# td-kwj-zp2023/webgpu-msm-bls12-377

Hardware: AMD Instinct MI355X
Metric: ms per 2^20 BLS12-377 G1 MSM (lower is better)
Workload: dtype u32 (29-bit limbs, 64-bit accumulate)

## Files before the change

webgpu-msm-bls12-377_amd/csrc/common.hpp:

```cpp
#pragma once
#include <stdint.h>

#include "../../include/msm377.h"

#ifndef MSM_HD
#if defined(__HIPCC__)
#include <hip/hip_runtime.h>
#define MSM_HD __host__ __device__ __forceinline__
#else
#define MSM_HD inline __attribute__((always_inline))
#endif
#endif

namespace msm377 {

constexpr uint32_t NB = 32768;
constexpr uint32_t NBIN = NB + 1;
constexpr uint32_t RP = NBIN + 1;
constexpr uint32_t PT_WORDS = 52;
constexpr uint32_t BKT_WORDS = 64;
constexpr uint32_t MAX_SORT_BLOCKS = 256;
constexpr uint32_t TREE_LEVELS = 15;
constexpr uint32_t SEG_MIN = 16;
constexpr uint32_t SEG_MAX = 128;
// ... 12 lines not shown
static_assert(short_windows(253, 15) == MSM377_NUM_WINDOWS && short_windows(253, NARROW_LOG) == NARROW_EVEN_WINDOWS, "at full width: the window counts of the main and the narrow path");

constexpr uint32_t NRANGE = 256;
constexpr uint32_t KRANGE = NB / NRANGE;
constexpr uint32_t KEY_TRACKED = 0x80000000u;
constexpr uint32_t KEY_UNSIGNED = 0x40000000u;
constexpr uint32_t SMALL_SORT_MAX = 1u << 16;
constexpr uint32_t SMALL_BINS_MAX = (1u << 12) + 1;
struct SortElem {
  uint32_t idx_sign;
  uint32_t key;
};
struct SortElem4 {
  uint32_t v;
};
constexpr uint32_t SORT_IDX_BITS = 23, SORT_SUB_BITS = 8;
constexpr uint64_t SORT_PACKED_MAX_COLUMNS = 1ull << SORT_IDX_BITS;
static_assert(SORT_IDX_BITS + SORT_SUB_BITS + 1 == 32, "index, sub and sign fill the 32-bit element");
static_assert(KRANGE < (1u << SORT_SUB_BITS), "sub = 0..KRANGE fits its field");
MSM_HD SortElem4 sort_pack(uint32_t idx, uint32_t sign, uint32_t sub) { return SortElem4{(sign << 31) | (sub << SORT_IDX_BITS) | idx}; }
MSM_HD uint32_t sort_sub(SortElem4 e) { return (e.v >> SORT_IDX_BITS) & ((1u << SORT_SUB_BITS) - 1u); }
MSM_HD uint32_t sort_idx_sign(SortElem4 e) { return e.v & ~(((1u << SORT_SUB_BITS) - 1u) << SORT_IDX_BITS); }
MSM_HD uint32_t range_first_key(uint32_t rg, uint32_t shift) { return rg * (KRANGE >> shift); }
inline uint32_t sort_elem_bytes(uint64_t columns, bool wide) { return (!wide && columns <= SORT_PACKED_MAX_COLUMNS) ? 4u : 8u; }

struct WorkItem {
  uint32_t row;
  uint32_t seg;
};
constexpr uint32_t META_BLOCK_WORDS = 2 * SEG_BINS + 4 + MSM377_NUM_WINDOWS;
constexpr size_t SLOT_WORDS = (size_t)MAX_WINDOW_SLOTS * MSM377_G1_PARTIAL_POINTS * MSM377_G1_POINT_WORDS;

constexpr uint32_t AFF_THREADS = 256, AFF_K = 8, AFF_BLOCK_POINTS = AFF_THREADS * AFF_K;
constexpr uint32_t AFF_STASH_WORDS = 52;
inline uint32_t affine_blocks(uint64_t n) { return (uint32_t)((n + AFF_BLOCK_POINTS - 1) / AFF_BLOCK_POINTS); }

constexpr uint32_t ACC_FLAG_WORD = 4;
constexpr uint32_t EVEN_FROM = 13;
constexpr uint32_t even_offset(uint32_t w) { return 16 * w - (w > EVEN_FROM ? w - EVEN_FROM : 0u); }
static_assert(even_offset(13) == 208 && even_offset(14) == 223 && even_offset(15) == 238 && even_offset(16) == 253, "13 x 16 + 3 x 15 = 253 bits");
constexpr uint32_t WIDE_BITS = MSM377_WIDE_WINDOW_BITS;
constexpr uint32_t WIDE_LOG = 19;
constexpr uint32_t WIDE_WINDOWS = 13;
constexpr uint32_t WIDE_FULL = 6;
constexpr uint32_t wide_width(uint32_t w) { return w < WIDE_FULL ? WIDE_BITS : WIDE_BITS - 1; }
constexpr uint32_t wide_offset(uint32_t w) { return w <= WIDE_FULL ? WIDE_BITS * w : WIDE_BITS * WIDE_FULL + (WIDE_BITS - 1) * (w - WIDE_FULL); }
static_assert(wide_offset(WIDE_WINDOWS - 1) == 234 && wide_offset(WIDE_WINDOWS - 1) + wide_width(WIDE_WINDOWS - 1) == 253, "the windows cover a 253-bit scalar");
constexpr uint32_t WIDE_NRANGE = 4096;
constexpr uint32_t WIDE_POINTS = WIDE_LOG + 1;
static_assert((1u << WIDE_LOG) == WIDE_NRANGE * KRANGE, "ranges of KRANGE keys cover the wide bucket set");
static_assert((1u << WIDE_LOG) <= MSM377_NUM_WINDOWS * NB, "the wide bucket set fits the main path's bucket, row and work-list buffers");
static_assert(WIDE_POINTS * 1 <= MAX_WINDOW_SLOTS * MSM377_G1_PARTIAL_POINTS, "the wide window record fits a partial-record slot");

constexpr uint32_t G1_REC_WORDS = 32;
constexpr uint32_t GLV_WINDOWS = MSM377_GLV_WINDOWS;

}
```

webgpu-msm-bls12-377_amd/csrc/consts_gen.hpp:

```cpp
#pragma once
#include <stdint.h>

namespace msm377 {

struct G1Consts {
static constexpr int NL = 13;
static constexpr int RS = 14;
static constexpr uint32_t KP2[13] = {0x20000002u, 0x308bffffu, 0x20000041u, 0x2d7510bfu, 0x290002e0u, 0x222fba08u, 0x3c78f79au, 0x3cc03d43u, 0x363445b2u, 0x26ca1492u, 0x231d82dfu, 0x3f1443aau, 0x35c748c1u};
static constexpr uint32_t KP6[13] = {0x20000006u, 0x31a3ffffu, 0x200000c6u, 0x285f323fu, 0x3b0008a3u, 0x268f2e1au, 0x356ae6d0u, 0x3640b7cdu, 0x229cd11au, 0x345e3dbau, 0x2958889fu, 0x3d3ccb00u, 0xa155da47u};
static constexpr uint32_t KP4W3[13] = {0x60000004u, 0x6117fffdu, 0x60000082u, 0x7aea217du, 0x720005bfu, 0x645f740fu, 0x78f1ef33u, 0x79807a86u, 0x6c688b64u, 0x6d942924u, 0x663b05bdu, 0x7e288753u, 0x6b8e9182u};
static constexpr uint32_t MOD2[13] = {0x00000002u, 0x108c0000u, 0x00000042u, 0x0d7510c0u, 0x090002e1u, 0x022fba09u, 0x1c78f79bu, 0x1cc03d44u, 0x163445b3u, 0x06ca1493u, 0x031d82e0u, 0x1f1443abu, 0x35c748c2u};
static constexpr uint32_t MOD4[13] = {0x00000004u, 0x01180000u, 0x00000085u, 0x1aea2180u, 0x120005c2u, 0x045f7412u, 0x18f1ef36u, 0x19807a89u, 0x0c688b67u, 0x0d942927u, 0x063b05c0u, 0x1e288756u, 0x6b8e9185u};
static constexpr uint32_t MOD[13] = {0x00000001u, 0x08460000u, 0x00000021u, 0x16ba8860u, 0x14800170u, 0x1117dd04u, 0x0e3c7bcdu, 0x1e601ea2u, 0x1b1a22d9u, 0x03650a49u, 0x118ec170u, 0x0f8a21d5u, 0x1ae3a461u};
static constexpr uint32_t ONE[13] = {0x19eaf730u, 0x171ffffeu, 0x0d714cf8u, 0x044e31d8u, 0x1eb6e262u, 0x0bfad163u, 0x00d46e9cu, 0x10b6ddbfu, 0x13b9cbddu, 0x075782afu, 0x03bd1d8au, 0x1557cab6u, 0x15742a14u};
static constexpr uint32_t R2[13] = {0x1c14cc5cu, 0x07b8df46u, 0x04c74875u, 0x0d6832fau, 0x05f4afc1u, 0x11ea1ee5u, 0x09265a5fu, 0x09fa84f9u, 0x12f6f558u, 0x18644b2bu, 0x1caa9452u, 0x011db07du, 0x0ef492d1u};
static constexpr uint32_t GEN_X[13] = {0x1ce797d8u, 0x17fe48a3u, 0x1f3536a5u, 0x0dc25c2bu, 0x1e104e6bu, 0x1eae505du, 0x0e4e1ad8u, 0x06034dddu, 0x1a0c4bbau, 0x1a00fcf3u, 0x0d60a010u, 0x0f8b893du, 0x0350969fu};
static constexpr uint32_t GEN_Y[13] = {0x1cad4e90u, 0x1ad19703u, 0x05ab84b1u, 0x0efc4cdcu, 0x0ea1dd3du, 0x16ca39d3u, 0x1a70f7f0u, 0x07c10e01u, 0x119daf26u, 0x1ea6b705u, 0x1f2b10a9u, 0x09c00e16u, 0x157eb1a4u};
static constexpr uint32_t B3[13] = {0x0dc0e58eu, 0x14d3fffcu, 0x0853e6a7u, 0x1f7584c9u, 0x1324a444u, 0x01c0ba22u, 0x0604543au, 0x15645bf8u, 0x04f91de4u, 0x0f3c737bu, 0x0819d5beu, 0x00f31c77u, 0x0a95357bu};
static constexpr uint32_t BETA[13] = {0x1c8a7893u, 0x0b7d08f2u, 0x06b88506u, 0x162aa2edu, 0x1c5fdf80u, 0x11b95a22u, 0x03b86dd7u, 0x1191f770u, 0x10701220u, 0x1501c11fu, 0x1cee88bbu, 0x118d05ecu, 0x06f2fa26u};
static constexpr uint32_t TE_S[13] = {0x08449ac2u, 0x16bc6341u, 0x1f27346eu, 0x003fa706u, 0x16341794u, 0x0e03035eu, 0x1f0a2ed9u, 0x0c4c0908u, 0x1a0645ffu, 0x0dd41749u, 0x078fb647u, 0x1b5db1c4u, 0x1660c39du};
static constexpr uint32_t TE_CS[13] = {0x0c11be99u, 0x0aedb353u, 0x14c24473u, 0x198caca0u, 0x1709c799u, 0x1d5780a3u, 0x0f7d035fu, 0x121a0ad5u, 0x0cb37c72u, 0x1eef061fu, 0x0da87607u, 0x1503504au, 0x001d4357u};
static constexpr uint32_t TE_2D[13] = {0x114806b1u, 0x04ef4e0du, 0x07df1bf4u, 0x01a7deddu, 0x07626a98u, 0x061c00c8u, 0x1b3f730cu, 0x037d439du, 0x1c957daau, 0x096f1594u, 0x098747aeu, 0x19dba77fu, 0x03dbbc1fu};
static constexpr uint32_t TE_INV_D[13] = {0x1235813du, 0x1a6958e8u, 0x0842a642u, 0x0ccc3277u, 0x130f1cf2u, 0x012ee262u, 0x18833f19u, 0x19503cf9u, 0x194bf957u, 0x1e6caec8u, 0x17390a9eu, 0x1ab4def3u, 0x10163111u};
static constexpr uint32_t TE_SR[13] = {0x15c55a01u, 0x1bcf91e7u, 0x09410bb6u, 0x1b458877u, 0x1f3e06b9u, 0x1b799510u, 0x13b0477au, 0x166cebb0u, 0x16d99580u, 0x1e1e3f33u, 0x141fe804u, 0x0e8bd79bu, 0x07643ddau};
static constexpr uint32_t TE_CSR[13] = {0x0e6d2f3fu, 0x083d0045u, 0x1a1e3b24u, 0x1500eeabu, 0x0b424b4au, 0x0f2708c5u, 0x13fa6b3eu, 0x0e79a13bu, 0x1bd40692u, 0x15a4c276u, 0x029c52e0u, 0x17b697c3u, 0x042252f1u};
static constexpr uint32_t TE_SBR[13] = {0x17d64e6fu, 0x0c701d9au, 0x1096c343u, 0x0f28269au, 0x1dd6a07bu, 0x0d2d995au, 0x0b7abebcu, 0x01039476u, 0x0754bb75u, 0x17ed77a6u, 0x10ad99d1u, 0x0295f06bu, 0x0eee0d30u};
static constexpr uint32_t TE_CSBR[13] = {0x101ae105u, 0x14e123bau, 0x0c011795u, 0x1e120f1bu, 0x013e4a5du, 0x00f36391u, 0x05460450u, 0x1213a321u, 0x02049adcu, 0x1e46b54eu, 0x03ec2c28u, 0x0719faedu, 0x04062136u};
static constexpr uint32_t CHK_RHS_RAW[13] = {0x1b151a26u, 0x1887416bu, 0x12ef1461u, 0x11a8bb6fu, 0x1402fb5bu, 0x08e38166u, 0x0355b0e6u, 0x1233c29au, 0x08a7a722u, 0x009a7635u, 0x1e0bf740u, 0x0c427686u, 0x0fde33f9u};
static constexpr uint32_t IMPORT_MONT384[13] = {0x00400000u, 0x00000000u, 0x00000000u, 0x00000000u, 0x00000000u, 0x00000000u, 0x00000000u, 0x00000000u, 0x00000000u, 0x00000000u, 0x00000000u, 0x00000000u, 0x00000000u};
static constexpr uint32_t TO64[13] = {0x1fffff68u, 0x166fffffu, 0x1fffec40u, 0x013f06ffu, 0x13ff2514u, 0x19d4c53eu, 0x0c167df6u, 0x16edcf8cu, 0x087b4e97u, 0x1c01e427u, 0x133d256fu, 0x05fbe934u, 0x08d6661eu};
static constexpr int PM2_NW = 12;
static constexpr uint32_t PM2_W[12] = {0xffffffffu, 0x8508bfffu, 0x30000000u, 0x170b5d44u, 0xba094800u, 0x1ef3622fu, 0x00f5138fu, 0x1a22d9f3u, 0x6ca1493bu, 0xc63b05c0u, 0x17c510eau, 0x01ae3a46u};
static constexpr uint32_t GEN_WIRE[24] = {0xb21be9efu, 0xeab9b16eu, 0xffcd394eu, 0xd5481512u, 0xbd37cb5cu, 0x188282c8u, 0xaa9d41bbu, 0x85951e2cu, 0xbf87ff54u, 0xc8fc6225u, 0xfe740a67u, 0x008848deu, 0x559c8ea6u, 0xfd82de55u, 0x34a9591au, 0xc2fe3d36u, 0x4fb82305u, 0x6d182ad4u, 0xca3e52d9u, 0xbd7fb348u, 0x30afeec4u, 0x1f674f5du, 0xc5102effu, 0x01914a69u};
};

struct GlvConsts {
static constexpr uint32_t LAMBDA[4] = {0x00000000u, 0x0a118000u, 0x90000001u, 0x452217ccu};
static constexpr uint32_t MU[9] = {0x7b820d29u, 0x5cc5a03bu, 0x6f25c6b5u, 0x3366fc87u, 0xaf90182cu, 0x7f72ed32u, 0x9fd37160u, 0xb3f7aa96u, 0x00000003u};
};

struct EdConsts {
static constexpr int NL = 9;
static constexpr int RS = 9;
static constexpr uint32_t KP2[9] = {0x20000002u, 0x2117ffffu, 0x20000084u, 0x29dbfb3fu, 0x36002b34u, 0x2d1e5c36u, 0x2ab305a1u, 0x37a68b28u, 0x002556c9u};
static constexpr uint32_t KP6[9] = {0x20000006u, 0x2347ffffu, 0x2000018eu, 0x3d93f1bfu, 0x2200819eu, 0x275b14a6u, 0x201910e6u, 0x26f3a17bu, 0x0070045fu};
static constexpr uint32_t KP4W3[9] = {0x60000004u, 0x622ffffdu, 0x60000107u, 0x73b7f67du, 0x6c005667u, 0x7a3cb86cu, 0x75660b41u, 0x6f4d164fu, 0x004aad92u};
static constexpr uint32_t MOD2[9] = {0x00000002u, 0x01180000u, 0x00000085u, 0x09dbfb40u, 0x16002b35u, 0x0d1e5c37u, 0x0ab305a2u, 0x17a68b29u, 0x002556cau};
static constexpr uint32_t MOD4[9] = {0x00000004u, 0x02300000u, 0x0000010au, 0x13b7f680u, 0x0c00566au, 0x1a3cb86fu, 0x15660b44u, 0x0f4d1652u, 0x004aad95u};
static constexpr uint32_t MOD[9] = {0x00000001u, 0x108c0000u, 0x00000042u, 0x14edfda0u, 0x1b00159au, 0x068f2e1bu, 0x155982d1u, 0x0bd34594u, 0x0012ab65u};
static constexpr uint32_t ONE[9] = {0x1ffffe4au, 0x1077ffffu, 0x1fff8e31u, 0x10d0103fu, 0x0ddb0965u, 0x07071c5cu, 0x18da2e10u, 0x0486f3a3u, 0x000ec090u};
static constexpr uint32_t R2[9] = {0x0615ebc3u, 0x1d9b570cu, 0x191f15fbu, 0x00f6d3e2u, 0x15ede530u, 0x0fadbc68u, 0x0428942fu, 0x06a15030u, 0x000c9478u};
static constexpr uint32_t ED_D[9] = {0x1febc5efu, 0x0eb3ffffu, 0x1abe9217u, 0x003be85fu, 0x0004720du, 0x05dec129u, 0x1512d0bbu, 0x09975a7cu, 0x000242cau};
static constexpr uint32_t ED_2D[9] = {0x1fd78bdeu, 0x1d67ffffu, 0x157d242eu, 0x0077d0bfu, 0x0008e41au, 0x0bbd8252u, 0x0a25a176u, 0x132eb4f9u, 0x00048594u};
static constexpr uint32_t GEN_X[9] = {0x0cca7270u, 0x0e8466dcu, 0x18ea02c5u, 0x0a3e1cacu, 0x0d288491u, 0x08fdc59du, 0x02b87f4fu, 0x00370735u, 0x0002b438u};
static constexpr uint32_t GEN_Y[9] = {0x19e7fa03u, 0x1cbf8d15u, 0x147cb8ddu, 0x0759f755u, 0x096d8529u, 0x0350b3f2u, 0x14b6ec89u, 0x0691eb12u, 0x000577c8u};
static constexpr uint32_t TE_2D[9] = {0x1fd78bdeu, 0x1d67ffffu, 0x157d242eu, 0x0077d0bfu, 0x0008e41au, 0x0bbd8252u, 0x0a25a176u, 0x132eb4f9u, 0x00048594u};
static constexpr uint32_t IMPORT_MONT256[9] = {0x00000020u, 0x00000000u, 0x00000000u, 0x00000000u, 0x00000000u, 0x00000000u, 0x00000000u, 0x00000000u, 0x00000000u};
static constexpr uint32_t TO64[9] = {0x1ffffff3u, 0x08e3ffffu, 0x1ffffc9fu, 0x0fea1edfu, 0x00fee725u, 0x0abaa896u, 0x0a745b60u, 0x06457773u, 0x000d4bdau};
static constexpr int PM2_NW = 8;
static constexpr uint32_t PM2_W[8] = {0xffffffffu, 0x0a117fffu, 0xd0000001u, 0x59aa76feu, 0x5c37b001u, 0x60b44d1eu, 0x9a2ca556u, 0x12ab655eu};
// ... 41 lines not shown
```

webgpu-msm-bls12-377_amd/csrc/context.hip:

```cpp
#include "context.hpp"

#include <string.h>

#include <algorithm>
#include <new>

#include "sequencer.hpp"

using namespace msm377;

hipError_t Resources::alloc(void** p, size_t bytes) {
  const hipError_t rc = hipMalloc(p, bytes);
  if (rc == hipSuccess) device.push_back(*p);
  else *p = nullptr;
  return rc;
}
hipError_t Resources::alloc_pinned(void** p, size_t bytes, unsigned flags) {
  const hipError_t rc = hipHostMalloc(p, bytes, flags);
  if (rc == hipSuccess) pinned.push_back(*p);
  else *p = nullptr;
  return rc;
}
hipError_t Resources::event(hipEvent_t* e, unsigned flags) {
  const hipError_t rc = hipEventCreateWithFlags(e, flags);
// ... 54 lines not shown
  ctx->tail_pool.wait_limit_ns = (int64_t)knobs.tail_wait_ms * 1000000ll;
  ctx->tail_pool.numa_local = knobs.tail_numa;
  Resources& own = ctx->own;
  const uint64_t cap = max_points;
  int prio_least = 0, prio_greatest = 0;
  bool ok = hipSetDevice(device) == hipSuccess;
  if (ok && hipDeviceGetStreamPriorityRange(&prio_least, &prio_greatest) != hipSuccess) prio_least = prio_greatest = 0;
  ok = ok && own.stream(&ctx->stream, &prio_greatest) == hipSuccess && own.stream(&ctx->stream2, &prio_least) == hipSuccess &&
       own.event(&ctx->bases_ready, hipEventDisableTiming) == hipSuccess;
  auto dalloc = [&](void** p, size_t bytes) { ok = ok && own.alloc(p, bytes) == hipSuccess; };
  if (!borrows_bases) dalloc((void**)&ctx->d_raw_points, cap * 96);
  dalloc((void**)&ctx->d_raw_scalars, cap * 32);
  if (!borrows_bases) dalloc((void**)&ctx->d_bases, 2 * cap * G1_REC_WORDS * 4);
  const uint64_t wcap = std::max<uint64_t>((uint64_t)MSM377_NUM_WINDOWS * cap, (uint64_t)NARROW_EVEN_WINDOWS * std::min<uint64_t>(cap, SMALL_SORT_MAX));
  dalloc((void**)&ctx->d_digits, wcap * 2);
  dalloc((void**)&ctx->d_range_counts, (size_t)NRANGE * MAX_SORT_BLOCKS * 4);
  dalloc((void**)&ctx->d_region_base, (size_t)MSM377_NUM_WINDOWS * (NRANGE + 1) * 4);
  dalloc((void**)&ctx->d_sort_temp, cap * MSM377_NUM_WINDOWS * sizeof(SortElem));
  dalloc((void**)&ctx->d_row_ptr, (size_t)MSM377_NUM_WINDOWS * RP * 4);
  dalloc((void**)&ctx->d_val_idx, wcap * 4);
  dalloc((void**)&ctx->d_buckets, (size_t)MSM377_NUM_WINDOWS * BKT_WORDS * NB * 4);
  dalloc((void**)&ctx->d_partials, (size_t)2 * SLOT_WORDS * 4);
  const uint64_t extra_items = std::max<uint64_t>((uint64_t)MSM377_NUM_WINDOWS * cap / SEG_MIN, (uint64_t)NARROW_EVEN_WINDOWS * std::min<uint64_t>(cap, SMALL_SORT_MAX) / NARROW_SEG) + 2;
  dalloc((void**)&ctx->d_work, ((size_t)MSM377_NUM_WINDOWS * NB + extra_items) * sizeof(WorkItem));
  dalloc((void**)&ctx->d_work_meta, (size_t)META_BLOCK_WORDS * 4);
  dalloc((void**)&ctx->d_row_ovf_base, (size_t)MSM377_NUM_WINDOWS * NB * 4);
  dalloc((void**)&ctx->d_split_rows, (size_t)MSM377_NUM_WINDOWS * NB * 4);
  dalloc((void**)&ctx->d_ovf, (size_t)extra_items * BKT_WORDS * 4);
  AffineConvert& aff = ctx->aff;
  ZeroCopyOut& zc = ctx->zc;
  const size_t aff_blocks = (size_t)affine_blocks(cap) + 1;
  dalloc((void**)&aff.d_count, 64);
  ok = ok && hipMemset(aff.d_count, 0, 64) == hipSuccess;
  dalloc((void**)&aff.d_stash, (size_t)affine_blocks(cap) * AFF_BLOCK_POINTS * AFF_STASH_WORDS * 4);
  dalloc((void**)&aff.d_trees, aff_blocks * 2 * AFF_THREADS * 13 * 4);
  const unsigned host_flags = hipHostMallocMapped | hipHostMallocCoherent;
  ok = ok && own.alloc_pinned((void**)&aff.h_prod, aff_blocks * 48, host_flags) == hipSuccess &&
       own.alloc_pinned((void**)&aff.h_inv, aff_blocks * 48, host_flags) == hipSuccess &&
       own.alloc_pinned((void**)&aff.h_flag, 64, host_flags) == hipSuccess &&
       hipHostGetDevicePointer((void**)&aff.dm_prod, aff.h_prod, 0) == hipSuccess &&
       hipHostGetDevicePointer((void**)&aff.dm_inv, aff.h_inv, 0) == hipSuccess &&
       hipHostGetDevicePointer((void**)&aff.dm_flag, aff.h_flag, 0) == hipSuccess &&
       own.event(&aff.up_done, hipEventDisableTiming) == hipSuccess;
  if (ok) aff.scratch.resize(aff_blocks);
  dalloc((void**)&ctx->d_err, 4 * sizeof(int));
  ok = ok && own.alloc_pinned((void**)&ctx->h_partials, (size_t)2 * SLOT_WORDS * 4, host_flags) == hipSuccess &&
       hipHostGetDevicePointer((void**)&zc.dm_partials, ctx->h_partials, 0) == hipSuccess &&
       own.alloc_pinned((void**)&zc.h_flag, 64, host_flags) == hipSuccess &&
       hipHostGetDevicePointer((void**)&zc.dm_flag, zc.h_flag, 0) == hipSuccess;
  if (ok) memset(zc.h_flag, 0, 64);
  dalloc((void**)&zc.d_count, 64);
  ok = ok && hipMemset(zc.d_count, 0, 64) == hipSuccess;
  ok = ok && own.alloc_pinned((void**)&ctx->h_err, 2 * sizeof(int)) == hipSuccess;
  for (int k = 0; ok && k < 2; k++) ok = ok && own.event(&ctx->done_ev[k], hipEventDisableTiming) == hipSuccess;
  for (int s = 0; ok && s < MSM377_NUM_STAGES; s++)
    for (int k = 0; k < 2; k++) ok = ok && own.event(&ctx->ev[s][k]) == hipSuccess;
  if (!ok) {
    ctx_destroy(ctx);
    return MSM377_ENOMEM;
  }
  *out = ctx;
  return MSM377_OK;
}

void ctx_destroy(msm377_ctx* ctx) {
  if (!ctx) return;
  ctx->tail_pool.shutdown();
// ... 66 lines not shown
```

webgpu-msm-bls12-377_amd/csrc/context.hpp:

```cpp
#pragma once
#include <hip/hip_runtime.h>

#include <functional>
#include <string>
#include <vector>

#include "common.hpp"
#include "fp64_host.hpp"
#include "knobs.hpp"
#include "tail_pool.hpp"

using msm377::SortElem;
using msm377::WorkItem;
using msm377::TailPool;
using msm377::Fp64;
using msm377::MAX_WINDOW_SLOTS;
using msm377::NARROW_SEG;
using msm377::Knobs;

struct Resources {
  std::vector<void*> device, pinned;
  std::vector<hipEvent_t> events;
  std::vector<hipStream_t> streams;
  hipError_t alloc(void** p, size_t bytes);
// ... 58 lines not shown
  uint32_t k = 0;
  int width = 0;
  uint32_t* tables = nullptr;
  bool valid() const { return k != 0; }
};

struct WideBuffers {
  uint32_t* digits = nullptr;
  SortElem* temp = nullptr;
  uint32_t* counts = nullptr;
  uint64_t cap = 0;
  bool ensure(Resources& own, uint64_t n, size_t counts_words);
  void release(Resources& own);
};

struct StageLayout {
  bool valid = false;
  msm377_stage_info info = {};
  const void* d_digits = nullptr;
  const uint32_t* d_key_max = nullptr;
  uint32_t coord_words = 16, limbs = 13;
};

struct BasesLayout {
  bool valid = false;
  msm377_bases_info info = {};
  const uint32_t* d_records = nullptr;
  const uint32_t* d_flagged = nullptr;
};


struct AffineConvert {
  uint32_t* d_stash = nullptr;
  uint32_t* d_trees = nullptr;
  uint32_t* h_prod = nullptr;
  uint32_t* h_inv = nullptr;
  uint32_t* h_flag = nullptr;
  uint32_t *dm_prod = nullptr, *dm_inv = nullptr, *dm_flag = nullptr;
  uint32_t* d_count = nullptr;
  hipEvent_t up_done = nullptr;
  std::vector<Fp64::El> scratch;
};

struct ZeroCopyOut {
  bool active = false;
  uint32_t out_seq = 0;
  uint32_t acc_seq = 0;
  uint32_t* h_flag = nullptr;
  uint32_t* dm_flag = nullptr;
  uint32_t* dm_partials = nullptr;
  uint32_t* d_count = nullptr;
};

struct NativeImport {
  uint64_t cap = 0;
  uint8_t* d_native = nullptr;
  uint32_t* d_inf_mask = nullptr;
  hipEvent_t import_done = nullptr;
  size_t mask_words() const { return (size_t)(((cap + 31) / 32 + 3) & ~3ull); }
  size_t points_bytes() const { return ((size_t)cap * 104 + 15) & ~(size_t)15; }
  uint8_t* native_points() const { return d_native; }
  uint8_t* native_scalars() const { return d_native + points_bytes(); }
};

struct HostStaging {
  uint8_t* h_stage = nullptr;
// ... 87 lines not shown
```

webgpu-msm-bls12-377_amd/csrc/kernels/convert.hpp:

```cpp
#pragma once
#include "../curves.hpp"

namespace msm377 {
namespace {


__global__ void __launch_bounds__(256) k_clear_words(uint32_t* __restrict__ a, uint32_t na, uint32_t* __restrict__ b, uint32_t nb) {
  for (uint32_t i = threadIdx.x; i < na; i += 256) a[i] = 0;
  for (uint32_t i = threadIdx.x; i < nb; i += 256) b[i] = 0;
}

template <class CV>
__global__ void __launch_bounds__(256) k_convert_bases(const uint32_t* __restrict__ raw, uint32_t* __restrict__ bases, uint64_t n, int* __restrict__ err) {
  uint64_t i = (uint64_t)blockIdx.x * 256 + threadIdx.x;
  if (i >= n) return;
  uint32_t w[CV::RAW_WORDS];
  load_words16(raw + i * CV::RAW_WORDS, w, CV::RAW_WORDS / 4);
  uint32_t o[CV::REC_WORDS];
  if (CV::convert(w, o)) atomicOr(err, ERR_TE_CONVERT);
  uint4* dst = reinterpret_cast<uint4*>(bases + i * CV::REC_WORDS);
#pragma unroll
  for (int k = 0; k < (int)CV::REC_WORDS / 4; k++) dst[k] = make_uint4(o[4 * k], o[4 * k + 1], o[4 * k + 2], o[4 * k + 3]);
}

// ... 12 lines not shown
  const uint32_t* raw;
  __device__ __forceinline__ bool load(uint64_t i, Fp::El& n1, Fp::El& n2, Fp::El& z) const {
    using K = G1Consts;
    uint32_t w[24];
    load_words16(raw + i * 24, w, 6);
    const Fp::El xr = Fp::from_words<12>(w), yr = Fp::from_words<12>(w + 12);
    const Fp::El u = Fp::add_lz(Fp::mul_lz(xr, Fp::from_const(K::TE_SR)), Fp::from_const(K::TE_S));
    const Fp::El v = Fp::mul_lz(yr, Fp::from_const(K::TE_SR));
    const Fp::El cu = Fp::csub(Fp::norm(Fp::add_lz(Fp::mul_lz(xr, Fp::from_const(K::TE_CSR)), Fp::from_const(K::TE_CS))), K::MOD);
    const Fp::El up = Fp::add_lz(u, Fp::one());
    z = Fp::mul_lz(up, v);
    n1 = Fp::mul_lz(up, cu);
    n2 = Fp::norm(Fp::add_kp_sub_sub2(z, K::KP4W3, Fp::zero(), v));
    return Te377::is_zero_mod_p(z);
  }
};
struct AffDoublingSource {
  const uint32_t* prev;
  uint32_t bits;
  __device__ __forceinline__ bool load(uint64_t i, Fp::El& n1, Fp::El& n2, Fp::El& z) const {
    Te377::Ext p = Te377::from_base_affine(TeAffBase::load_base(prev, (uint32_t)i), false);
    bool bad = false;
#pragma unroll 1
    for (uint32_t k = 0; k < bits; k++) {
      p = Te377::add(p, p);
      bad |= Te377::is_bad(p);
    }
    n1 = Fp::canon(p.x);
    n2 = Fp::canon(p.y);
    z = Fp::canon(p.z);
    return bad;
  }
};
template <class SRC>
__global__ void __launch_bounds__(AFF_THREADS, 4) k_affine_up(SRC src, uint64_t n, uint32_t* __restrict__ stash,
                                                              uint32_t* __restrict__ trees, uint32_t* __restrict__ block_prod, uint32_t* __restrict__ host_flag, uint32_t* __restrict__ dev_count,
                                                              int* __restrict__ err, uint32_t prio) {
  if (prio) __builtin_amdgcn_s_setprio(3);
  using K = G1Consts;
  __shared__ uint32_t tree[2 * AFF_THREADS][13];
  const uint32_t tid = threadIdx.x, blk = blockIdx.x;
  const uint64_t base = (uint64_t)blk * AFF_BLOCK_POINTS + tid;
  bool bad = false;
  Fp::El c = Fp::one();
#pragma unroll 1
  for (uint32_t j = 0; j < AFF_K; j++) {
    const uint64_t i = base + (uint64_t)j * AFF_THREADS;
    if (i >= n) break;
    Fp::El n1, n2, z;
    if (src.load(i, n1, n2, z)) {
      bad = true;
      z = Fp::one();
    }
    uint32_t o[AFF_STASH_WORDS];
    put13(o, n1);
    put13(o + 13, n2);
    put13(o + 26, z);
    put13(o + 39, c);
    uint4* dst = reinterpret_cast<uint4*>(stash) + ((size_t)blk * AFF_K + j) * (AFF_STASH_WORDS / 4) * AFF_THREADS + tid;
#pragma unroll
    for (int k = 0; k < (int)AFF_STASH_WORDS / 4; k++) dst[(size_t)k * AFF_THREADS] = make_uint4(o[4 * k], o[4 * k + 1], o[4 * k + 2], o[4 * k + 3]);
    c = Fp::mul_lz(c, z);
  }
  if (bad) atomicOr(err, ERR_TE_CONVERT);
  put13(tree[AFF_THREADS + tid], c);
  for (uint32_t size = AFF_THREADS / 2; size >= 1; size >>= 1) {
    __syncthreads();
    if (tid < size) put13(tree[size + tid], Fp::mul_lz(get13(tree[2 * (size + tid)]), get13(tree[2 * (size + tid) + 1])));
  }
  __syncthreads();
  uint32_t* out = trees + (size_t)blk * (2 * AFF_THREADS * 13);
  const uint32_t* flat = &tree[0][0];
  for (uint32_t k = tid; k < 2 * AFF_THREADS * 13; k += AFF_THREADS) out[k] = flat[k];
  if (tid == 0) {
    const Fp::El root = Fp::mul(get13(tree[1]), Fp::from_const(K::TO64));
    uint32_t w[12];
    Fp::to_words<12>(root, w);
#pragma unroll
    for (int j = 0; j < 12; j++) block_prod[(size_t)blk * 12 + j] = w[j];
    __threadfence_system();
    if (atomicAdd(dev_count, 1u) == gridDim.x - 1) {
      *dev_count = 0;
      __threadfence_system();
      *reinterpret_cast<volatile uint32_t*>(host_flag) = gridDim.x;
    }
  }
}

__global__ void __launch_bounds__(AFF_THREADS, 2) k_affine_down(uint64_t n, const uint32_t* __restrict__ stash, const uint32_t* __restrict__ trees,
                                                                const uint32_t* __restrict__ block_inv, uint32_t* __restrict__ bases, uint32_t prio) {
  if (prio) __builtin_amdgcn_s_setprio(3);
  __shared__ uint32_t tree[2 * AFF_THREADS][13];
  const uint32_t tid = threadIdx.x, blk = blockIdx.x;
  const uint32_t* in = trees + (size_t)blk * (2 * AFF_THREADS * 13);
  uint32_t* flat = &tree[0][0];
  for (uint32_t k = tid; k < 2 * AFF_THREADS * 13; k += AFF_THREADS) flat[k] = in[k];
  __syncthreads();
  if (tid == 0) {
    uint32_t w[12];
#pragma unroll
    for (int j = 0; j < 12; j++) w[j] = block_inv[(size_t)blk * 12 + j];
    put13(tree[1], Fp::from_words<12>(w));
  }
  for (uint32_t size = 1; size < AFF_THREADS; size <<= 1) {
    __syncthreads();
    if (tid < size) {
      const uint32_t k = size + tid;
      const Fp::El inv_k = get13(tree[k]), a = get13(tree[2 * k]), b = get13(tree[2 * k + 1]);
      put13(tree[2 * k], Fp::mul_lz(inv_k, b));
      put13(tree[2 * k + 1], Fp::mul_lz(inv_k, a));
    }
  }
  __syncthreads();
  Fp::El inv = get13(tree[AFF_THREADS + tid]);
  const uint64_t base = (uint64_t)blk * AFF_BLOCK_POINTS + tid;
#pragma unroll 1
  for (int j = (int)AFF_K - 1; j >= 0; j--) {
    const uint64_t i = base + (uint64_t)j * AFF_THREADS;
    if (i >= n) continue;
    uint32_t w[AFF_STASH_WORDS];
    {
      const uint4* src = reinterpret_cast<const uint4*>(stash) + ((size_t)blk * AFF_K + j) * (AFF_STASH_WORDS / 4) * AFF_THREADS + tid;
#pragma unroll
      for (int k = 0; k < (int)AFF_STASH_WORDS / 4; k++) {
        const uint4 v = src[(size_t)k * AFF_THREADS];
        w[4 * k + 0] = v.x;
        w[4 * k + 1] = v.y;
        w[4 * k + 2] = v.z;
        w[4 * k + 3] = v.w;
      }
    }
    const Fp::El zi = Fp::mul_lz(inv, get13(w + 39));
    inv = Fp::mul_lz(inv, get13(w + 26));
    const Fp::El x = Fp::mul(get13(w), zi), y = Fp::mul(get13(w + 13), zi);
    const Fp::El ymx = Fp::sub(y, x), ypx = Fp::add(y, x), kt = Fp::mul_lz(Fp::mul_lz(x, y), Fp::from_const(G1Consts::TE_2D));
    uint32_t o[TeAffBase::REC_WORDS];
    put13(o, ymx);
    put13(o + 13, ypx);
    put13(o + 26, kt);
    o[39] = 0;
    uint4* dst = reinterpret_cast<uint4*>(bases + i * TeAffBase::REC_WORDS);
#pragma unroll
    for (int k = 0; k < (int)TeAffBase::REC_WORDS / 4; k++) dst[k] = make_uint4(o[4 * k], o[4 * k + 1], o[4 * k + 2], o[4 * k + 3]);
  }
}


__global__ void __launch_bounds__(256) k_convert_bases_glv(const uint32_t* __restrict__ raw, uint32_t* __restrict__ bases, uint64_t n) {
  uint64_t i = (uint64_t)blockIdx.x * 256 + threadIdx.x;
  if (i >= n) return;
  uint32_t w[24];
  load_words16(raw + i * 24, w, 6);
  const Fp::El x = Fp::to_mont(Fp::from_words<12>(w));
  const Fp::El y = Fp::to_mont(Fp::from_words<12>(w + 12));
  const Fp::El bx = Fp::mul(x, Fp::from_const(G1Consts::BETA));
  constexpr uint32_t REC_WORDS = G1Dev::REC_WORDS;
  uint32_t o[REC_WORDS];
#pragma unroll
  for (int j = 0; j < 13; j++) {
    o[j] = x.l[j];
    o[13 + j] = y.l[j];
  }
#pragma unroll
  for (int j = 26; j < 32; j++) o[j] = 0;
  uint4* dst = reinterpret_cast<uint4*>(bases + i * REC_WORDS);
#pragma unroll
  for (int k = 0; k < 8; k++) dst[k] = make_uint4(o[4 * k], o[4 * k + 1], o[4 * k + 2], o[4 * k + 3]);
#pragma unroll
  for (int j = 0; j < 13; j++) o[j] = bx.l[j];
  dst = reinterpret_cast<uint4*>(bases + (n + i) * REC_WORDS);
#pragma unroll
  for (int k = 0; k < 8; k++) dst[k] = make_uint4(o[4 * k], o[4 * k + 1], o[4 * k + 2], o[4 * k + 3]);
}


}
}
```

webgpu-msm-bls12-377_amd/csrc/sequencer.hip:

```cpp
#include "sequencer.hpp"

#include <hip/hip_runtime.h>
#include <string.h>

#include <algorithm>
#include <atomic>
#include <chrono>
#include <functional>
#include <initializer_list>
#include <thread>
#include <type_traits>
#include <vector>

#include "context.hpp"
#include "host_tail.hpp"
#include "ed_batch_mul_host.hpp"
#include "validate_host.hpp"
#include "kernels/accumulate.hpp"
#include "kernels/batch_mul.hpp"
#include "kernels/batch_mul_multi.hpp"
#include "kernels/ed_batch_mul.hpp"
#include "kernels/commit_rows.hpp"
#include "kernels/convert.hpp"
#include "kernels/decompose.hpp"
// ... 118 lines not shown
  b.valid = true;
  ctx->last.bases = b;
}
template <class CV>
constexpr uint32_t bases_form_of() {
  return std::is_same<CV, TeDev>::value ? MSM377_BASES_TE_PROJECTIVE : std::is_same<CV, EdDev>::value ? MSM377_BASES_ED : MSM377_BASES_WEIERSTRASS;
}

template <class CV>
int convert_bases(msm377_ctx* ctx, const uint32_t* d_raw, uint64_t n, uint64_t first = 0, bool clear_err = true) {
  if (n == 0) return MSM377_OK;
  if (ctx->timing == 1) (void)hipEventRecord(ctx->ev[MSM377_STAGE_CONVERT][0], ctx->stream2);
  if (clear_err) hipLaunchKernelGGL(k_clear_words, dim3(1), dim3(256), 0, ctx->stream2, (uint32_t*)(ctx->d_err + 2), 1u, (uint32_t*)nullptr, 0u);
  hipLaunchKernelGGL(k_convert_bases<CV>, dim3((unsigned)((n + 255) / 256)), dim3(256), 0, ctx->stream2, d_raw, ctx->d_bases + first * CV::REC_WORDS, n,
                     ctx->d_err + 2);
  HIP_TRY(ctx, hipGetLastError());
  note_bases(ctx, bases_form_of<CV>(), ctx->d_bases, n, first);
  if (ctx->timing == 1) (void)hipEventRecord(ctx->ev[MSM377_STAGE_CONVERT][1], ctx->stream2);
  HIP_TRY(ctx, hipEventRecord(ctx->bases_ready, ctx->stream2));
  return MSM377_OK;
}

int affine_convert_begin(msm377_ctx* ctx, const uint32_t* d_raw, uint64_t n, const uint32_t* prev_window_records = nullptr, uint32_t doublings = 0,
                         bool clear_err = true) {
  if (n == 0) return MSM377_OK;
  const uint32_t nblk = affine_blocks(n);
  if (ctx->timing == 1) (void)hipEventRecord(ctx->ev[MSM377_STAGE_CONVERT][0], ctx->stream2);
  __atomic_store_n(ctx->aff.h_flag, 0u, __ATOMIC_RELEASE);
  if (clear_err) hipLaunchKernelGGL(k_clear_words, dim3(1), dim3(256), 0, ctx->stream2, (uint32_t*)(ctx->d_err + 2), 1u, (uint32_t*)nullptr, 0u);
  if (prev_window_records)
    hipLaunchKernelGGL(k_affine_up<AffDoublingSource>, dim3(nblk), dim3(AFF_THREADS), 0, ctx->stream2, AffDoublingSource{prev_window_records, doublings}, n,
                       ctx->aff.d_stash, ctx->aff.d_trees, ctx->aff.dm_prod, ctx->aff.dm_flag, ctx->aff.d_count, ctx->d_err + 2, ctx->knobs.conv_wave_prio);
  else
    hipLaunchKernelGGL(k_affine_up<AffWireSource>, dim3(nblk), dim3(AFF_THREADS), 0, ctx->stream2, AffWireSource{d_raw}, n, ctx->aff.d_stash, ctx->aff.d_trees,
                       ctx->aff.dm_prod, ctx->aff.dm_flag, ctx->aff.d_count, ctx->d_err + 2, ctx->knobs.conv_wave_prio);
  HIP_TRY(ctx, hipGetLastError());
  HIP_TRY(ctx, hipEventRecord(ctx->aff.up_done, ctx->stream2));
  if (ctx->knobs.tail_threads > 1 && nblk >= 32) ctx->tail_pool.prewake(ctx->knobs.aff_prewake_us, std::min(ctx->knobs.tail_threads, TailPool::WORKERS + 1) - 1);
  return MSM377_OK;
}

int affine_convert_finish(msm377_ctx* ctx, uint32_t* d_records_out, uint64_t n) {
  if (n == 0) return MSM377_OK;
  const uint32_t nblk = affine_blocks(n);
  const auto t0 = std::chrono::steady_clock::now();
  for (uint32_t spins = 0; __atomic_load_n(ctx->aff.h_flag, __ATOMIC_ACQUIRE) != nblk; spins++) {
    __builtin_ia32_pause();
    if ((spins & 0xfff) == 0xfff && std::chrono::steady_clock::now() - t0 > std::chrono::milliseconds(20)) {
      HIP_TRY(ctx, hipEventSynchronize(ctx->aff.up_done));
      break;
    }
  }
  if (__atomic_load_n(ctx->aff.h_flag, __ATOMIC_ACQUIRE) != nblk) {
    ctx->err = "batched affine conversion: the block products did not arrive";
    return MSM377_EHIP;
  }
  {
    const int inv_rc = invert_block_products_mt(ctx, 0, nblk);
    ctx->tail_pool.disarm();
    if (inv_rc) return inv_rc;
  }
  hipLaunchKernelGGL(k_affine_down, dim3(nblk), dim3(AFF_THREADS), 0, ctx->stream2, n, ctx->aff.d_stash, ctx->aff.d_trees, ctx->aff.dm_inv, d_records_out, ctx->knobs.conv_wave_prio);
  HIP_TRY(ctx, hipGetLastError());
  note_bases(ctx, MSM377_BASES_TE_AFFINE, d_records_out, n);
  if (ctx->timing == 1) (void)hipEventRecord(ctx->ev[MSM377_STAGE_CONVERT][1], ctx->stream2);
  HIP_TRY(ctx, hipEventRecord(ctx->bases_ready, ctx->stream2));
  return MSM377_OK;
}

uint32_t auto_seg(const msm377_ctx* ctx, uint64_t entries, bool glv) {
  const uint32_t forced = glv ? ctx->knobs.seg_glv : ctx->knobs.seg_plain;
  if (forced) return forced;
  const uint64_t s = ((entries >> 18) + 7) & ~7ull;
  return (uint32_t)std::min<uint64_t>(std::max<uint64_t>(s, SEG_MIN), SEG_MAX);
}


enum Recode { RECODE_EQUAL16, RECODE_EVEN16, RECODE_NARROW22, RECODE_SHORT, RECODE_WIDE13, RECODE_GLV8 };
enum TailKind { TE_TAIL, XYZZ_TAIL, ED_TAIL };
struct WindowPlan {
  Recode recode = RECODE_EQUAL16;
  uint32_t slots = MSM377_NUM_WINDOWS;
  uint32_t bucket_log = MSM377_WINDOW_BITS - 1;
  const uint32_t* table = nullptr;
  uint64_t table_stride = 0;
  const uint32_t* bases_override = nullptr;
  uint32_t short_bytes = 0, short_bits = 0;
  TailKind tail = TE_TAIL;
  bool on_caller = false;
  int records = MSM377_NUM_WINDOWS;
  int short_from = 0;
  int cbits() const { return (int)bucket_log + 1; }
  int planes() const { return (int)bucket_log; }
};

// ... 2110 lines not shown
```

Baseline: 2.336.

## Specialize wire-source affine conversion to stash fewer words and recompute from raw input

Adds dedicated up/down kernels for the wire-input path of batched affine conversion. The up kernel keeps only the denominator product and the running prefix (28 words) instead of four field elements (52 words), and the down kernel reloads the raw point and recomputes the Edwards coordinates using new constants. This cuts stash write and read traffic and uses a cheaper single-denominator formulation, at the cost of reading the raw input twice and the register pressure implied by the lower launch-bounds occupancy hint.

```diff
diff --git a/webgpu-msm-bls12-377_amd/csrc/common.hpp b/webgpu-msm-bls12-377_amd/csrc/common.hpp
--- a/webgpu-msm-bls12-377_amd/csrc/common.hpp
+++ b/webgpu-msm-bls12-377_amd/csrc/common.hpp
@@ -68,7 +68,8 @@
 constexpr size_t SLOT_WORDS = (size_t)MAX_WINDOW_SLOTS * MSM377_G1_PARTIAL_POINTS * MSM377_G1_POINT_WORDS;
 
 constexpr uint32_t AFF_THREADS = 256, AFF_K = 8, AFF_BLOCK_POINTS = AFF_THREADS * AFF_K;
-constexpr uint32_t AFF_STASH_WORDS = 52;
+constexpr uint32_t AFF_STASH_WORDS = 28;
+constexpr uint32_t AFF_TABLE_STASH_WORDS = 52;
 inline uint32_t affine_blocks(uint64_t n) { return (uint32_t)((n + AFF_BLOCK_POINTS - 1) / AFF_BLOCK_POINTS); }
 
 constexpr uint32_t ACC_FLAG_WORD = 4;
diff --git a/webgpu-msm-bls12-377_amd/csrc/consts_gen.hpp b/webgpu-msm-bls12-377_amd/csrc/consts_gen.hpp
--- a/webgpu-msm-bls12-377_amd/csrc/consts_gen.hpp
+++ b/webgpu-msm-bls12-377_amd/csrc/consts_gen.hpp
@@ -26,6 +26,9 @@
 static constexpr uint32_t TE_CSR[13] = {0x0e6d2f3fu, 0x083d0045u, 0x1a1e3b24u, 0x1500eeabu, 0x0b424b4au, 0x0f2708c5u, 0x13fa6b3eu, 0x0e79a13bu, 0x1bd40692u, 0x15a4c276u, 0x029c52e0u, 0x17b697c3u, 0x042252f1u};
 static constexpr uint32_t TE_SBR[13] = {0x17d64e6fu, 0x0c701d9au, 0x1096c343u, 0x0f28269au, 0x1dd6a07bu, 0x0d2d995au, 0x0b7abebcu, 0x01039476u, 0x0754bb75u, 0x17ed77a6u, 0x10ad99d1u, 0x0295f06bu, 0x0eee0d30u};
 static constexpr uint32_t TE_CSBR[13] = {0x101ae105u, 0x14e123bau, 0x0c011795u, 0x1e120f1bu, 0x013e4a5du, 0x00f36391u, 0x05460450u, 0x1213a321u, 0x02049adcu, 0x1e46b54eu, 0x03ec2c28u, 0x0719faedu, 0x04062136u};
+static constexpr uint32_t TE_C[13] = {0x18d0ec00u, 0x19d5ac0bu, 0x099a00afu, 0x14f3163du, 0x15201f1au, 0x185e2df4u, 0x10000b58u, 0x16cc24d5u, 0x0cfaac7eu, 0x1feb43c4u, 0x0f6e64c6u, 0x1143d6d9u, 0x182ac132u};
+static constexpr uint32_t TE_B_RAW[13] = {0x109adc02u, 0x002c1256u, 0x071e9f27u, 0x17651e1cu, 0x064272e6u, 0x05b2fe0bu, 0x1690bf8bu, 0x0663068cu, 0x0e86ef0du, 0x10ae65fcu, 0x16505bb3u, 0x0c5a693cu, 0x032d7560u};
+static constexpr uint32_t TE_E_RAW[13] = {0x0f652401u, 0x0819eda9u, 0x18e160fau, 0x1f556a43u, 0x0e3d8e89u, 0x0b64def9u, 0x17abbc42u, 0x17fd1815u, 0x0c9333ccu, 0x12b6a44du, 0x1b3e65bcu, 0x032fb898u, 0x17b62f01u};
 static constexpr uint32_t CHK_RHS_RAW[13] = {0x1b151a26u, 0x1887416bu, 0x12ef1461u, 0x11a8bb6fu, 0x1402fb5bu, 0x08e38166u, 0x0355b0e6u, 0x1233c29au, 0x08a7a722u, 0x009a7635u, 0x1e0bf740u, 0x0c427686u, 0x0fde33f9u};
 static constexpr uint32_t IMPORT_MONT384[13] = {0x00400000u, 0x00000000u, 0x00000000u, 0x00000000u, 0x00000000u, 0x00000000u, 0x00000000u, 0x00000000u, 0x00000000u, 0x00000000u, 0x00000000u, 0x00000000u, 0x00000000u};
 static constexpr uint32_t TO64[13] = {0x1fffff68u, 0x166fffffu, 0x1fffec40u, 0x013f06ffu, 0x13ff2514u, 0x19d4c53eu, 0x0c167df6u, 0x16edcf8cu, 0x087b4e97u, 0x1c01e427u, 0x133d256fu, 0x05fbe934u, 0x08d6661eu};
diff --git a/webgpu-msm-bls12-377_amd/csrc/context.hip b/webgpu-msm-bls12-377_amd/csrc/context.hip
--- a/webgpu-msm-bls12-377_amd/csrc/context.hip
+++ b/webgpu-msm-bls12-377_amd/csrc/context.hip
@@ -110,7 +110,8 @@
   const size_t aff_blocks = (size_t)affine_blocks(cap) + 1;
   dalloc((void**)&aff.d_count, 64);
   ok = ok && hipMemset(aff.d_count, 0, 64) == hipSuccess;
-  dalloc((void**)&aff.d_stash, (size_t)affine_blocks(cap) * AFF_BLOCK_POINTS * AFF_STASH_WORDS * 4);
+  static_assert(AFF_STASH_WORDS <= AFF_TABLE_STASH_WORDS && AFF_STASH_WORDS % 4 == 0 && AFF_TABLE_STASH_WORDS % 4 == 0, "16-byte pieces");
+  dalloc((void**)&aff.d_stash, (size_t)affine_blocks(cap) * AFF_BLOCK_POINTS * AFF_TABLE_STASH_WORDS * 4);
   dalloc((void**)&aff.d_trees, aff_blocks * 2 * AFF_THREADS * 13 * 4);
   const unsigned host_flags = hipHostMallocMapped | hipHostMallocCoherent;
   ok = ok && own.alloc_pinned((void**)&aff.h_prod, aff_blocks * 48, host_flags) == hipSuccess &&
diff --git a/webgpu-msm-bls12-377_amd/csrc/context.hpp b/webgpu-msm-bls12-377_amd/csrc/context.hpp
--- a/webgpu-msm-bls12-377_amd/csrc/context.hpp
+++ b/webgpu-msm-bls12-377_amd/csrc/context.hpp
@@ -114,6 +114,7 @@
 
 struct AffineConvert {
   uint32_t* d_stash = nullptr;
+  const uint32_t* d_wire = nullptr;
   uint32_t* d_trees = nullptr;
   uint32_t* h_prod = nullptr;
   uint32_t* h_inv = nullptr;
diff --git a/webgpu-msm-bls12-377_amd/csrc/kernels/convert.hpp b/webgpu-msm-bls12-377_amd/csrc/kernels/convert.hpp
--- a/webgpu-msm-bls12-377_amd/csrc/kernels/convert.hpp
+++ b/webgpu-msm-bls12-377_amd/csrc/kernels/convert.hpp
@@ -68,6 +68,68 @@
     return bad;
   }
 };
+__device__ __forceinline__ void aff_tree_up(uint32_t (*tree)[13], const Fp::El& c, uint32_t* __restrict__ trees, uint32_t* __restrict__ block_prod,
+                                            uint32_t* __restrict__ host_flag, uint32_t* __restrict__ dev_count) {
+  const uint32_t tid = threadIdx.x, blk = blockIdx.x;
+  put13(tree[AFF_THREADS + tid], c);
+  for (uint32_t size = AFF_THREADS / 2; size >= 1; size >>= 1) {
+    __syncthreads();
+    if (tid < size) put13(tree[size + tid], Fp::mul_lz(get13(tree[2 * (size + tid)]), get13(tree[2 * (size + tid) + 1])));
+  }
+  __syncthreads();
+  uint32_t* out = trees + (size_t)blk * (2 * AFF_THREADS * 13);
+  const uint32_t* flat = &tree[0][0];
+  for (uint32_t k = tid; k < 2 * AFF_THREADS * 13; k += AFF_THREADS) out[k] = flat[k];
+  if (tid == 0) {
+    const Fp::El root = Fp::mul(get13(tree[1]), Fp::from_const(G1Consts::TO64));
+    uint32_t w[12];
+    Fp::to_words<12>(root, w);
+#pragma unroll
+    for (int j = 0; j < 12; j++) block_prod[(size_t)blk * 12 + j] = w[j];
+    __threadfence_system();
+    if (atomicAdd(dev_count, 1u) == gridDim.x - 1) {
+      *dev_count = 0;
+      __threadfence_system();
+      *reinterpret_cast<volatile uint32_t*>(host_flag) = gridDim.x;
+    }
+  }
+}
+__device__ __forceinline__ Fp::El aff_tree_down(uint32_t (*tree)[13], const uint32_t* __restrict__ trees, const uint32_t* __restrict__ block_inv) {
+  const uint32_t tid = threadIdx.x, blk = blockIdx.x;
+  const uint32_t* in = trees + (size_t)blk * (2 * AFF_THREADS * 13);
+  uint32_t* flat = &tree[0][0];
+  for (uint32_t k = tid; k < 2 * AFF_THREADS * 13; k += AFF_THREADS) flat[k] = in[k];
+  __syncthreads();
+  if (tid == 0) {
+    uint32_t w[12];
+#pragma unroll
+    for (int j = 0; j < 12; j++) w[j] = block_inv[(size_t)blk * 12 + j];
+    put13(tree[1], Fp::from_words<12>(w));
+  }
+  for (uint32_t size = 1; size < AFF_THREADS; size <<= 1) {
+    __syncthreads();
+    if (tid < size) {
+      const uint32_t k = size + tid;
+      const Fp::El inv_k = get13(tree[k]), a = get13(tree[2 * k]), b = get13(tree[2 * k + 1]);
+      put13(tree[2 * k], Fp::mul_lz(inv_k, b));
+      put13(tree[2 * k + 1], Fp::mul_lz(inv_k, a));
+    }
+  }
+  __syncthreads();
+  return get13(tree[AFF_THREADS + tid]);
+}
+__device__ __forceinline__ void aff_store_record(uint32_t* __restrict__ bases, uint64_t i, const Fp::El& x, const Fp::El& y) {
+  const Fp::El ymx = Fp::sub(y, x), ypx = Fp::add(y, x), kt = Fp::mul_lz(Fp::mul_lz(x, y), Fp::from_const(G1Consts::TE_2D));
+  uint32_t o[TeAffBase::REC_WORDS];
+  put13(o, ymx);
+  put13(o + 13, ypx);
+  put13(o + 26, kt);
+  o[39] = 0;
+  uint4* dst = reinterpret_cast<uint4*>(bases + i * TeAffBase::REC_WORDS);
+#pragma unroll
+  for (int k = 0; k < (int)TeAffBase::REC_WORDS / 4; k++) dst[k] = make_uint4(o[4 * k], o[4 * k + 1], o[4 * k + 2], o[4 * k + 3]);
+}
+
 template <class SRC>
 __global__ void __launch_bounds__(AFF_THREADS, 4) k_affine_up(SRC src, uint64_t n, uint32_t* __restrict__ stash,
                                                               uint32_t* __restrict__ trees, uint32_t* __restrict__ block_prod, uint32_t* __restrict__ host_flag, uint32_t* __restrict__ dev_count,
@@ -88,14 +150,14 @@
       bad = true;
       z = Fp::one();
     }
-    uint32_t o[AFF_STASH_WORDS];
+    uint32_t o[AFF_TABLE_STASH_WORDS];
     put13(o, n1);
     put13(o + 13, n2);
     put13(o + 26, z);
     put13(o + 39, c);
-    uint4* dst = reinterpret_cast<uint4*>(stash) + ((size_t)blk * AFF_K + j) * (AFF_STASH_WORDS / 4) * AFF_THREADS + tid;
-#pragma unroll
-    for (int k = 0; k < (int)AFF_STASH_WORDS / 4; k++) dst[(size_t)k * AFF_THREADS] = make_uint4(o[4 * k], o[4 * k + 1], o[4 * k + 2], o[4 * k + 3]);
+    uint4* dst = reinterpret_cast<uint4*>(stash) + ((size_t)blk * AFF_K + j) * (AFF_TABLE_STASH_WORDS / 4) * AFF_THREADS + tid;
+#pragma unroll
+    for (int k = 0; k < (int)AFF_TABLE_STASH_WORDS / 4; k++) dst[(size_t)k * AFF_THREADS] = make_uint4(o[4 * k], o[4 * k + 1], o[4 * k + 2], o[4 * k + 3]);
     c = Fp::mul_lz(c, z);
   }
   if (bad) atomicOr(err, ERR_TE_CONVERT);
@@ -154,11 +216,11 @@
   for (int j = (int)AFF_K - 1; j >= 0; j--) {
     const uint64_t i = base + (uint64_t)j * AFF_THREADS;
     if (i >= n) continue;
-    uint32_t w[AFF_STASH_WORDS];
+    uint32_t w[AFF_TABLE_STASH_WORDS];
     {
-      const uint4* src = reinterpret_cast<const uint4*>(stash) + ((size_t)blk * AFF_K + j) * (AFF_STASH_WORDS / 4) * AFF_THREADS + tid;
-#pragma unroll
-      for (int k = 0; k < (int)AFF_STASH_WORDS / 4; k++) {
+      const uint4* src = reinterpret_cast<const uint4*>(stash) + ((size_t)blk * AFF_K + j) * (AFF_TABLE_STASH_WORDS / 4) * AFF_THREADS + tid;
+#pragma unroll
+      for (int k = 0; k < (int)AFF_TABLE_STASH_WORDS / 4; k++) {
         const uint4 v = src[(size_t)k * AFF_THREADS];
         w[4 * k + 0] = v.x;
         w[4 * k + 1] = v.y;
@@ -181,6 +243,88 @@
   }
 }
 
+struct AffWirePoint {
+  Fp::El x, y;
+  __device__ __forceinline__ AffWirePoint(const uint32_t* __restrict__ raw, uint64_t i) {
+    uint32_t w[24];
+    load_words16(raw + i * 24, w, 6);
+    x = Fp::from_words<12>(w);
+    y = Fp::from_words<12>(w + 12);
+  }
+  __device__ __forceinline__ Fp::El a() const {
+    Fp::El r = x;
+    r.l[0] += 1;
+    return r;
+  }
+  __device__ __forceinline__ Fp::El b() const { return Fp::add_lz(x, Fp::from_const(G1Consts::TE_B_RAW)); }
+  __device__ __forceinline__ Fp::El e() const { return Fp::add_lz(x, Fp::from_const(G1Consts::TE_E_RAW)); }
+};
+
+__global__ void __launch_bounds__(AFF_THREADS, 2) k_affine_up_wire(const uint32_t* __restrict__ raw, uint64_t n, uint32_t* __restrict__ stash,
+                                                                   uint32_t* __restrict__ trees, uint32_t* __restrict__ block_prod, uint32_t* __restrict__ host_flag,
+                                                                   uint32_t* __restrict__ dev_count, int* __restrict__ err, uint32_t prio) {
+  if (prio) __builtin_amdgcn_s_setprio(3);
+  __shared__ uint32_t tree[2 * AFF_THREADS][13];
+  const uint32_t tid = threadIdx.x, blk = blockIdx.x;
+  const uint64_t base = (uint64_t)blk * AFF_BLOCK_POINTS + tid;
+  bool bad = false;
+  Fp::El c = Fp::one();
+#pragma unroll 1
+  for (uint32_t j = 0; j < AFF_K; j++) {
+    const uint64_t i = base + (uint64_t)j * AFF_THREADS;
+    if (i >= n) break;
+    const AffWirePoint pt(raw, i);
+    Fp::El d = Fp::mul_lz(pt.y, pt.b());
+    if (Te377::is_zero_mod_p(d)) {
+      bad = true;
+      d = Fp::one();
+    }
+    uint32_t o[AFF_STASH_WORDS];
+    put13(o, d);
+    put13(o + 13, c);
+    o[26] = o[27] = 0;
+    uint4* dst = reinterpret_cast<uint4*>(stash) + ((size_t)blk * AFF_K + j) * (AFF_STASH_WORDS / 4) * AFF_THREADS + tid;
+#pragma unroll
+    for (int k = 0; k < (int)AFF_STASH_WORDS / 4; k++) dst[(size_t)k * AFF_THREADS] = make_uint4(o[4 * k], o[4 * k + 1], o[4 * k + 2], o[4 * k + 3]);
+    c = Fp::mul_lz(c, d);
+  }
+  if (bad) atomicOr(err, ERR_TE_CONVERT);
+  aff_tree_up(tree, c, trees, block_prod, host_flag, dev_count);
+}
+
+__global__ void __launch_bounds__(AFF_THREADS, 2) k_affine_down_wire(const uint32_t* __restrict__ raw, uint64_t n, const uint32_t* __restrict__ stash,
+                                                                     const uint32_t* __restrict__ trees, const uint32_t* __restrict__ block_inv, uint32_t* __restrict__ bases,
+                                                                     uint32_t prio) {
+  if (prio) __builtin_amdgcn_s_setprio(3);
+  __shared__ uint32_t tree[2 * AFF_THREADS][13];
+  const uint32_t tid = threadIdx.x, blk = blockIdx.x;
+  Fp::El inv = aff_tree_down(tree, trees, block_inv);
+  const uint64_t base = (uint64_t)blk * AFF_BLOCK_POINTS + tid;
+#pragma unroll 1
+  for (int j = (int)AFF_K - 1; j >= 0; j--) {
+    const uint64_t i = base + (uint64_t)j * AFF_THREADS;
+    if (i >= n) continue;
+    uint32_t w[AFF_STASH_WORDS];
+    {
+      const uint4* src = reinterpret_cast<const uint4*>(stash) + ((size_t)blk * AFF_K + j) * (AFF_STASH_WORDS / 4) * AFF_THREADS + tid;
+#pragma unroll
+      for (int k = 0; k < (int)AFF_STASH_WORDS / 4; k++) {
+        const uint4 v = src[(size_t)k * AFF_THREADS];
+        w[4 * k + 0] = v.x;
+        w[4 * k + 1] = v.y;
+        w[4 * k + 2] = v.z;
+        w[4 * k + 3] = v.w;
+      }
+    }
+    const AffWirePoint pt(raw, i);
+    const Fp::El zi = Fp::mul_lz(inv, get13(w + 13));
+    inv = Fp::mul_lz(inv, get13(w));
+    const Fp::El y = Fp::mul(pt.e(), Fp::mul_lz(pt.y, zi));
+    const Fp::El x = Fp::mul(Fp::mul_lz(pt.a(), Fp::from_const(G1Consts::TE_C)), Fp::mul_lz(pt.b(), zi));
+    aff_store_record(bases, i, x, y);
+  }
+}
+
 
 __global__ void __launch_bounds__(256) k_convert_bases_glv(const uint32_t* __restrict__ raw, uint32_t* __restrict__ bases, uint64_t n) {
   uint64_t i = (uint64_t)blockIdx.x * 256 + threadIdx.x;
diff --git a/webgpu-msm-bls12-377_amd/csrc/sequencer.hip b/webgpu-msm-bls12-377_amd/csrc/sequencer.hip
--- a/webgpu-msm-bls12-377_amd/csrc/sequencer.hip
+++ b/webgpu-msm-bls12-377_amd/csrc/sequencer.hip
@@ -174,8 +174,9 @@
     hipLaunchKernelGGL(k_affine_up<AffDoublingSource>, dim3(nblk), dim3(AFF_THREADS), 0, ctx->stream2, AffDoublingSource{prev_window_records, doublings}, n,
                        ctx->aff.d_stash, ctx->aff.d_trees, ctx->aff.dm_prod, ctx->aff.dm_flag, ctx->aff.d_count, ctx->d_err + 2, ctx->knobs.conv_wave_prio);
   else
-    hipLaunchKernelGGL(k_affine_up<AffWireSource>, dim3(nblk), dim3(AFF_THREADS), 0, ctx->stream2, AffWireSource{d_raw}, n, ctx->aff.d_stash, ctx->aff.d_trees,
-                       ctx->aff.dm_prod, ctx->aff.dm_flag, ctx->aff.d_count, ctx->d_err + 2, ctx->knobs.conv_wave_prio);
+    hipLaunchKernelGGL(k_affine_up_wire, dim3(nblk), dim3(AFF_THREADS), 0, ctx->stream2, d_raw, n, ctx->aff.d_stash, ctx->aff.d_trees, ctx->aff.dm_prod,
+                       ctx->aff.dm_flag, ctx->aff.d_count, ctx->d_err + 2, ctx->knobs.conv_wave_prio);
+  ctx->aff.d_wire = prev_window_records ? nullptr : d_raw;
   HIP_TRY(ctx, hipGetLastError());
   HIP_TRY(ctx, hipEventRecord(ctx->aff.up_done, ctx->stream2));
   if (ctx->knobs.tail_threads > 1 && nblk >= 32) ctx->tail_pool.prewake(ctx->knobs.aff_prewake_us, std::min(ctx->knobs.tail_threads, TailPool::WORKERS + 1) - 1);
@@ -202,7 +203,11 @@
     ctx->tail_pool.disarm();
     if (inv_rc) return inv_rc;
   }
-  hipLaunchKernelGGL(k_affine_down, dim3(nblk), dim3(AFF_THREADS), 0, ctx->stream2, n, ctx->aff.d_stash, ctx->aff.d_trees, ctx->aff.dm_inv, d_records_out, ctx->knobs.conv_wave_prio);
+  if (ctx->aff.d_wire)
+    hipLaunchKernelGGL(k_affine_down_wire, dim3(nblk), dim3(AFF_THREADS), 0, ctx->stream2, ctx->aff.d_wire, n, ctx->aff.d_stash, ctx->aff.d_trees, ctx->aff.dm_inv,
+                       d_records_out, ctx->knobs.conv_wave_prio);
+  else
+    hipLaunchKernelGGL(k_affine_down, dim3(nblk), dim3(AFF_THREADS), 0, ctx->stream2, n, ctx->aff.d_stash, ctx->aff.d_trees, ctx->aff.dm_inv, d_records_out, ctx->knobs.conv_wave_prio);
   HIP_TRY(ctx, hipGetLastError());
   note_bases(ctx, MSM377_BASES_TE_AFFINE, d_records_out, n);
   if (ctx->timing == 1) (void)hipEventRecord(ctx->ev[MSM377_STAGE_CONVERT][1], ctx->stream2);
```

After: 2.395. 1.03x slower.
